# acg-team/ProGraphMSA

Measured on AMD Instinct MI355X. Metric: DP cell-updates/sec (GCUPS) + wall-clock on 256 seqs × 1000 aa, WAG, higher is better.
Workload: dtype f32

## Files before the change

### include/pgm_hip.h

```cpp
#ifndef PGM_HIP_H_
#define PGM_HIP_H_

#include <stdint.h>
#include <stddef.h>

#ifdef __cplusplus
extern "C" {
#endif

#define PGM_OK 0
#define PGM_ERR_INVALID 1
#define PGM_ERR_DEVICE 2
#define PGM_ERR_BACKTRACK 3
#define PGM_ERR_NOMEM 4

#define PGM_GAP 0xFFFFFFFFu


typedef struct pgm_graph {
    uint32_t n;
    uint32_t dim;
    const double *sites;
    const int32_t *e_rowptr;
    const uint32_t *e_col;
// ... 55 lines not shown
                               const pgm_graph *const *g2, const pgm_model *const *model,
                               const pgm_scores *scores, const pgm_site_ref *res1,
                               const pgm_site_ref *res2, pgm_align_out *out);
int pgm_align_batch_run(pgm_ctx *ctx, pgm_align_batch *b);
int pgm_align_batch_fetch(pgm_ctx *ctx, pgm_align_batch *b, pgm_align_out *out);
void pgm_align_batch_destroy(pgm_ctx *ctx, pgm_align_batch *b);
uint64_t pgm_align_batch_cells(const pgm_align_batch *b);
int pgm_align_batch_time(pgm_ctx *ctx, pgm_align_batch *b, int reps, float *ms_prep,
                         float *ms_emission, float *ms_fill, float *ms_traceback);
int pgm_align_batch_stage_times(pgm_align_batch *b, int reset, float *ms_prep, float *ms_emission, float *ms_fill,
                                uint32_t *launches);
int pgm_align_batch_job_times(pgm_ctx *ctx, pgm_align_batch *b, uint64_t *ticks);
int pgm_align_batch_test_stall(pgm_align_batch *b, uint32_t job, uint32_t band, uint32_t spin_limit);
int pgm_test_cu_shares(uint32_t cus, double lean_cost, uint32_t nlean, double band_cost, uint32_t nbands, double rest_cost,
                       uint32_t nrest, uint32_t ncrit, double longest_chain, uint32_t *out4);
int pgm_align_batch_read_matrices(pgm_ctx *ctx, pgm_align_batch *b, uint32_t job, float *M,
                                  float *X, float *Y, float *W, float *S);

int pgm_nw_pairs_batch(pgm_ctx *ctx, uint32_t dim, const int32_t *score, int32_t gap_open,
                       int32_t gap_extend, uint32_t nseq, const int8_t *syms,
                       const uint32_t *offs, uint32_t npairs, const uint32_t *pi,
                       const uint32_t *pj, int32_t *counts, uint32_t *gaps);
#define PGM_NW_REDUCED 1u
int pgm_nw_pairs_submit(pgm_ctx *ctx, uint32_t dim, const int32_t *score, int32_t gap_open,
                        int32_t gap_extend, uint32_t nseq, const int8_t *syms,
                        const uint32_t *offs, uint32_t npairs, const uint32_t *pi,
                        const uint32_t *pj, uint32_t flags, int32_t *counts, uint32_t *gaps, int *ticket);
int pgm_nw_pairs_wait(pgm_ctx *ctx, int ticket);
float pgm_nw_last_kernel_ms(pgm_ctx *ctx);
void *pgm_host_alloc(size_t bytes);
// ... 80 lines not shown
```

### prographmsa_amd/__init__.py

```python
import ctypes as C
import os

_HERE = os.path.dirname(os.path.abspath(__file__))
LIB_PATH = os.path.join(_HERE, "lib", "libpgm_hip.so")
PGMSA_PATH = os.path.join(_HERE, "bin", "pgmsa")

PGM_OK, PGM_ERR_INVALID, PGM_ERR_DEVICE, PGM_ERR_BACKTRACK, PGM_ERR_NOMEM = 0, 1, 2, 3, 4
PGM_GAP = 0xFFFFFFFF
PGM_BATCH_KEEP_MATRICES = 1
PGM_NW_REDUCED = 1
PGM_MERGE_RESIDENT = 1


class pgm_graph(C.Structure):
    _fields_ = [("n", C.c_uint32), ("dim", C.c_uint32), ("sites", C.POINTER(C.c_double)),
                ("e_rowptr", C.POINTER(C.c_int32)), ("e_col", C.POINTER(C.c_uint32)), ("e_val", C.POINTER(C.c_float)),
                ("r_rowptr", C.POINTER(C.c_int32)), ("r_col", C.POINTER(C.c_uint32)), ("r_units", C.POINTER(C.c_uint32))]


class pgm_model(C.Structure):
    _fields_ = [("M", C.POINTER(C.c_double)), ("pi", C.POINTER(C.c_double))]


class pgm_scores(C.Structure):
# ... 26 lines not shown
    _fields_ = [("masks", C.POINTER(C.c_uint64)), ("children", C.POINTER(C.c_uint32)), ("nleaves", C.c_uint32), ("ncols", C.c_uint32)]


class pgm_wls_job(C.Structure):
    _fields_ = [("label", C.POINTER(C.c_int8)), ("offset", C.POINTER(C.c_double)), ("nsub", C.c_uint32)]


class pgm_align_out(C.Structure):
    _fields_ = [("score", C.c_float), ("n_tr_indels", C.c_uint32), ("len", C.c_uint32), ("status", C.c_int32),
                ("map1", C.POINTER(C.c_uint32)), ("map2", C.POINTER(C.c_uint32))]


EXPORTS = [
    "pgm_device_count", "pgm_ctx_create", "pgm_ctx_destroy", "pgm_last_error", "pgm_ctx_device_info",
    "pgm_align_graphs_batch", "pgm_align_batch_create", "pgm_align_batch_create_ex", "pgm_align_batch_create_res", "pgm_align_graphs_batch_res", "pgm_align_batch_run", "pgm_align_batch_fetch",
    "pgm_align_batch_destroy", "pgm_align_batch_cells", "pgm_align_batch_test_stall", "pgm_test_cu_shares", "pgm_align_batch_stage_times", "pgm_align_batch_job_times", "pgm_align_batch_time", "pgm_align_batch_read_matrices",
    "pgm_nw_pairs_batch", "pgm_nw_pairs_submit", "pgm_nw_pairs_wait", "pgm_nw_last_kernel_ms", "pgm_host_alloc", "pgm_host_free", "pgm_csprofile_load", "pgm_csprofile_create_batch", "pgm_csprofile_create_batch_res",
    "pgm_csprofile_last_kernel_ms", "pgm_mldist_batch", "pgm_prealigned_counts_batch", "pgm_kmer_cosine", "pgm_dist_last_kernel_ms",
    "pgm_merge_profiles_batch", "pgm_merge_profiles_batch_ex", "pgm_resident_reset", "pgm_resident_onehot", "pgm_resident_import", "pgm_merge_last_kernel_ms",
    "pgm_gapmask_extend_batch", "pgm_gap_parsimony_batch", "pgm_parsimony_last_kernel_ms",
    "pgm_wls_load", "pgm_wls_pair_sums_batch", "pgm_wls_last_kernel_ms", "pgm_wls_last_launches",
]


def _load():
    if not os.path.exists(LIB_PATH):
        raise ImportError("libpgm_hip.so is not built (%s); run `python -c 'import __graft_entry__ as g; g.build()'` "
                          "— there is no CPU fallback for the hot path" % LIB_PATH)
    lib = C.CDLL(LIB_PATH)
    vp, u32, i32 = C.c_void_p, C.c_uint32, C.c_int32
    PG, PM = C.POINTER(C.POINTER(pgm_graph)), C.POINTER(C.POINTER(pgm_model))
# ... 2 lines not shown
        "pgm_ctx_create": (C.c_int, [C.c_int, C.POINTER(vp)]),
        "pgm_ctx_destroy": (None, [vp]),
        "pgm_last_error": (C.c_char_p, []),
        "pgm_ctx_device_info": (C.c_int, [vp, C.c_char_p, C.c_size_t, C.POINTER(C.c_int)]),
        "pgm_align_graphs_batch": (C.c_int, [vp, u32, PG, PG, PM, C.POINTER(pgm_scores), C.POINTER(pgm_align_out)]),
        "pgm_align_batch_create": (C.c_int, [vp, u32, PG, PG, PM, C.POINTER(pgm_scores), C.POINTER(vp)]),
        "pgm_align_batch_create_ex": (C.c_int, [vp, u32, PG, PG, PM, C.POINTER(pgm_scores), u32, C.POINTER(vp)]),
        "pgm_align_batch_create_res": (C.c_int, [vp, u32, PG, PG, PM, C.POINTER(pgm_scores), u32, C.POINTER(pgm_site_ref), C.POINTER(pgm_site_ref), C.POINTER(vp)]),
        "pgm_align_graphs_batch_res": (C.c_int, [vp, u32, PG, PG, PM, C.POINTER(pgm_scores), C.POINTER(pgm_site_ref), C.POINTER(pgm_site_ref), C.POINTER(pgm_align_out)]),
        "pgm_align_batch_run": (C.c_int, [vp, vp]),
        "pgm_align_batch_fetch": (C.c_int, [vp, vp, C.POINTER(pgm_align_out)]),
        "pgm_align_batch_destroy": (None, [vp, vp]),
        "pgm_align_batch_cells": (C.c_uint64, [vp]),
        "pgm_align_batch_test_stall": (C.c_int, [vp, u32, u32, u32]),
        "pgm_test_cu_shares": (C.c_int, [u32, C.c_double, u32, C.c_double, u32, C.c_double, u32, u32, C.c_double, C.POINTER(C.c_uint32)]),
        "pgm_align_batch_stage_times": (C.c_int, [vp, C.c_int] + [C.POINTER(C.c_float)] * 3 + [C.POINTER(u32)]),
        "pgm_align_batch_job_times": (C.c_int, [vp, vp, C.POINTER(C.c_uint64)]),
        "pgm_align_batch_time": (C.c_int, [vp, vp, C.c_int] + [C.POINTER(C.c_float)] * 4),
        "pgm_align_batch_read_matrices": (C.c_int, [vp, vp, u32] + [C.POINTER(C.c_float)] * 5),
        "pgm_nw_pairs_batch": (C.c_int, [vp, u32, C.POINTER(i32), i32, i32, u32, C.POINTER(C.c_int8), C.POINTER(u32), u32,
                                         C.POINTER(u32), C.POINTER(u32), C.POINTER(i32), C.POINTER(u32)]),
        "pgm_nw_pairs_submit": (C.c_int, [vp, u32, C.POINTER(i32), i32, i32, u32, C.POINTER(C.c_int8), C.POINTER(u32), u32,
                                          C.POINTER(u32), C.POINTER(u32), u32, C.POINTER(i32), C.POINTER(u32), C.POINTER(C.c_int)]),
        "pgm_nw_pairs_wait": (C.c_int, [vp, C.c_int]),
        "pgm_host_alloc": (vp, [C.c_size_t]),
        "pgm_host_free": (None, [vp]),
        "pgm_nw_last_kernel_ms": (C.c_float, [vp]),
        "pgm_csprofile_load": (C.c_int, [vp, u32, u32] + [C.POINTER(C.c_double)] * 3),
        "pgm_csprofile_create_batch": (C.c_int, [vp, u32, C.POINTER(C.c_int8), C.POINTER(u32)] + [C.POINTER(C.c_double)] * 4
                                       + [C.POINTER(C.c_uint64)]),
# ... 63 lines not shown
```

### prographmsa_amd/csrc/pgm_align_kernels.h

```cpp
#ifndef PGM_ALIGN_KERNELS_H_
#define PGM_ALIGN_KERNELS_H_

#include <hip/hip_runtime.h>
#include <math.h>
#include <type_traits>
#include "pgm_device.h"

#define PGM_NEG_INF (-INFINITY)

__device__ __forceinline__ float pgm_ls_log_add(float x, float add) {
    const float a = 2.44247459618085927548717403238913328776812604856113966238617812902399112761292613763080658235564f;
    const float b = -4.2040783745848554315883301529007786406310628696382695994938550046831869207082846248658671f;
    const float c = -0.72123729809042963774358701619456664388406302428056983119308906451199556380646306f;
    const uint32_t bits = __float_as_uint(x);
    const float e = (float)((int32_t)(bits >> 23) - 126);
    const float d = __uint_as_float(((bits << 9) >> 9) ^ 0x3f000000u);
    float t = __fdiv_rn(b, __fsub_rn(d, c));
    const float u = __fadd_rn(e, a);
    t = __fadd_rn(t, add);
    t = __fadd_rn(t, u);
    return t;
}

__device__ __forceinline__ float pgm_emission_finish(float num, float ay, float bx, float match_init) {
// ... 138 lines not shown
    return ((size_t)b * J.tsteps + (x + l)) * 64u + l;
}
__device__ __forceinline__ float4 pgm_load_cell(const PgmJob &J, uint32_t y, uint32_t x) {
    return J.cells[pgm_cell_index(J, y, x)];
}

__device__ __forceinline__ float pgm_dpp_wave_shr1(float src, float lane0_value) {
    return __int_as_float(__builtin_amdgcn_update_dpp(__float_as_int(lane0_value), __float_as_int(src), 0x138, 0xf, 0xf, false));
}

#define PGM_GLOBAL __attribute__((address_space(1)))
typedef float pgm_v4f __attribute__((ext_vector_type(4)));
template <class T> __device__ __forceinline__ T pgm_gld(const T *p) { return *(const PGM_GLOBAL T *)(uintptr_t)p; }
#define PGM_EM_TB 4
template <int DP, int RB>
__global__ void __launch_bounds__(4 * PGM_ROWS) pgm_emission_skew_kernel(const PgmJob *__restrict__ jobs) {
    typedef float pgm_v2f __attribute__((ext_vector_type(2)));
    constexpr int NT = DP / 4;
    constexpr int COLS = 64 + PGM_EM_TB * PGM_BLOCK - PGM_HALO - 1;
    constexpr int STR = DP + 1;
    __shared__ pgm_v2f tp[(COLS + 1) * STR];
    __shared__ float bq[COLS];
    const PgmJob &J = jobs[blockIdx.z];
    const uint32_t tb0 = blockIdx.x * PGM_EM_TB;
    const uint32_t rsh = J.rshift, nvb = J.nb << rsh;
    if (tb0 >= J.nblk || 4u * RB * blockIdx.y >= nvb) return;
    if (J.tabhdr && pgm_gld(J.tabhdr) == 0) return;
    auto row_of = [&](uint32_t v, uint32_t lane_) { return ((((v >> rsh) << 6) + lane_) << rsh) | (v & ((1u << rsh) - 1u)); };
    auto sblock_of = [&](uint32_t v, uint32_t tb_) { return ((((size_t)(v >> rsh) * J.nblk + tb_) << rsh) | (v & ((1u << rsh) - 1u))); };
    const uint32_t t0 = tb0 * PGM_BLOCK;
    const int cbase = (int)t0 - 63;
    if ((DP == 20 || DP == 4) && RB == 1) {
        constexpr int TE = DP + 1;
        float *const tab = (float *)tp;
        static_assert(COLS * TE <= (COLS + 1) * STR * 2, "score table must fit the column staging area");
        static_assert(DP > 20 || TE <= 32, "row classes must fit As");
        __shared__ float As[32];
        const uint32_t fb0 = 4u * blockIdx.y + threadIdx.x / PGM_ROWS;
// ... 2395 lines not shown
```

### prographmsa_amd/csrc/pgm_capi.hip

```cpp
#include <hip/hip_runtime.h>

#include <algorithm>
#include <cmath>
#include <cstdio>
#include <thread>
#include <atomic>
#include <chrono>
#include <queue>
#include <cstdlib>
#include <cstring>
#include <numeric>
#include <mutex>
#include <string>
#include <unordered_set>
#include <vector>
#include <sys/mman.h>

#include "pgm_align_kernels.h"
#include "pgm_crit_kernels.h"
#include "pgm_nw_kernels.h"
#include "pgm_csprofile_kernels.h"
#include "pgm_dist_kernels.h"
#include "pgm_merge_kernels.h"
#include "pgm_parsimony_kernels.h"
// ... 116 lines not shown
    PgmItem *d_items = nullptr;
    uint32_t *d_lean = nullptr;
    uint32_t nlean = 0, nlean_workers = 0;
    uint32_t nbands = 0, nband_workers = 0;
    uint32_t nbands_narrow = 0, nwide_workers = 0;
    PgmItem *d_bands = nullptr;
    unsigned long long *d_times = nullptr;
    hipEvent_t ev_join_b = nullptr;
    bool crit_c3 = false, rest_c3 = false;
    uint32_t ncrit = 0, ncrit_workers = 0, ntb_c = 0;
    hipEvent_t ev_join_c = nullptr;
    uint32_t ntb_b = 0, ntb_b_workers = 0;
    uint32_t lq_off = 0, ntb = 0, ntb_workers = 0;
    int2 *d_tblist = nullptr;
    hipEvent_t ev_fork = nullptr, ev_join = nullptr;
    uint32_t test_spin_limit = 0, test_stall_job = 0xFFFFFFFFu, test_stall_band = 0;
    double acc_ms[3] = {0, 0, 0};
    uint32_t acc_n = 0;
    bool ev_pending = false;
    uint32_t nitems = 0;
    uint32_t nworkers = 0, maxnblk = 0;
    PgmJob *d_jobs = nullptr;
    uint32_t *d_order = nullptr;
    int *d_tabhdr = nullptr;
    size_t in_bytes = 0, work_bytes = 0, cell_bytes = 0, out_bytes = 0;
    std::vector<size_t> res_off, map1_off, map2_off;
    hipEvent_t ev[5] = {nullptr, nullptr, nullptr, nullptr, nullptr};
};

extern "C" {
// ... 362 lines not shown
        ctx->sc_host[slot] = nullptr; ctx->sc_host_bytes[slot] = 0;
        const size_t want = bytes + bytes / 4;
        hipError_t e = pinned_alloc(want, &ctx->sc_host[slot]);
        if (e != hipSuccess) return e;
        ctx->sc_host_bytes[slot] = want;
    }
    *out = ctx->sc_host[slot];
    return hipSuccess;
}
static hipError_t scratch_events(pgm_ctx *ctx) {
    for (int k = 0; k < 2; ++k)
        if (!ctx->sc_ev[k]) { hipError_t e = hipEventCreate(&ctx->sc_ev[k]); if (e != hipSuccess) return e; }
    return hipSuccess;
}

struct CuShares { uint32_t lean, band, crit, rest, rest_need; double t_goal, fl, fb; };
static CuShares cu_shares(uint32_t cus, double lean_cost, uint32_t nlean, double band_cost, uint32_t nbands, double rest_cost, uint32_t nrest, uint32_t ncrit, double rsweep) {
    CuShares r = {0u, 0u, 0u, 0u, 0u, 0.0, 1.0, 1.0};
    cus = std::max(1u, cus);
    const uint32_t queues = (nlean != 0) + (nbands != 0) + (nrest != 0);
    if (ncrit != 0 && cus > queues) r.crit = std::min(std::min(ncrit, cus / 2u), cus - queues);
    const uint32_t cap = std::max(1u, cus - r.crit);
    const double sum = (nlean ? lean_cost : 0.0) + (nbands ? band_cost : 0.0) + (nrest ? rest_cost : 0.0);
    const double t_par = std::max(1e-3, sum / cap);
    r.t_goal = std::max(std::max(rsweep, t_par), 1e-3);
    const double w = std::min(1.0, std::max(0.0, (rsweep / t_par - 1.0) / 0.5));
    r.fl = 1.0 - 0.4 * w; r.fb = 1.0 - 0.25 * w;
    auto need = [](double cost, double t, uint32_t most) { return (uint32_t)std::min<double>(most, std::max(1.0, std::ceil(cost / t))); };
    const uint32_t band_most = (nbands + PGM_WAVES - 1) / PGM_WAVES;
    uint32_t lean = nlean ? need(lean_cost, r.fl * r.t_goal, nlean) : 0u, band = nbands ? need(band_cost, r.fb * r.t_goal, band_most) : 0u;
    uint32_t rest = nrest ? need(rest_cost, r.t_goal, nrest) : 0u;
    if (lean + band + rest > cap) {
        const double scale = (double)cap / (double)(lean + band + rest);
        auto cut = [&](uint32_t v) { return v ? std::max(1u, (uint32_t)std::floor(v * scale)) : 0u; };
        lean = cut(lean); band = cut(band); rest = cut(rest);
        while (lean + band + rest > cap) {
            uint32_t *big = &rest; if (band > *big) big = &band; if (lean > *big) big = &lean;
            if (*big <= 1u) break;
            --*big;
        }
    }
    r.rest_need = rest;
    const uint32_t left = cap > lean + band + rest ? cap - lean - band - rest : 0u;
    if (nrest) rest = std::min(nrest, rest + left);
    else if (nbands) band = std::min(band_most, band + left);
    else if (nlean) lean = std::min(nlean, lean + left);
// ... 15 lines not shown
    hipError_t e;
    for (uint32_t i = 0; i < b->njobs; ++i) ((PgmJob::Result *)(b->h_out + b->res_off[i]))->status = PGM_STATUS_PENDING;
    if (timed && (e = hipEventRecord(b->ev[0], s)) != hipSuccess) return e;
    if (b->maxdim <= 4) {
        const size_t prep_lds = ((size_t)b->maxdim * b->maxdim + b->maxdim + 256 * ((size_t)b->maxdim + 1)) * sizeof(float);
        hipLaunchKernelGGL((pgm_prep_kernel<4, 256>), dim3(b->njobs, 2, (b->maxn + 255) / 256), dim3(256), prep_lds, s, b->d_jobs, b->d_sync, (uint32_t)b->sync_ints);
    } else if (b->maxdim <= 20) {
        const size_t prep_lds = ((size_t)b->maxdim * b->maxdim + b->maxdim + 256 * ((size_t)b->maxdim + 1)) * sizeof(float);
        hipLaunchKernelGGL((pgm_prep_kernel<20, 256>), dim3(b->njobs, 2, (b->maxn + 255) / 256), dim3(256), prep_lds, s, b->d_jobs, b->d_sync, (uint32_t)b->sync_ints);
    } else {
        const size_t prep_lds = ((size_t)b->maxdim * b->maxdim + b->maxdim + 64 * ((size_t)b->maxdim + 1)) * sizeof(float);
        hipLaunchKernelGGL((pgm_prep_kernel<64, 64>), dim3(b->njobs, 2, (b->maxn + 63) / 64), dim3(64), prep_lds, s, b->d_jobs, b->d_sync, (uint32_t)b->sync_ints);
    }
    if ((e = hipGetLastError()) != hipSuccess) return e;
    if (timed && (e = hipEventRecord(b->ev[1], s)) != hipSuccess) return e;
    const dim3 eg((b->maxnblk + PGM_EM_TB - 1) / PGM_EM_TB, (b->maxnb + 3) / 4, b->njobs);
    if (b->maxdim <= 4) hipLaunchKernelGGL((pgm_emission_skew_kernel<4, 1>), eg, dim3(4 * PGM_ROWS), 0, s, b->d_jobs);
    else if (b->maxdim <= 20) hipLaunchKernelGGL((pgm_emission_skew_kernel<20, 1>), eg, dim3(4 * PGM_ROWS), 0, s, b->d_jobs);
    else hipLaunchKernelGGL((pgm_emission_skew_kernel<64, 1>), eg, dim3(4 * PGM_ROWS), 0, s, b->d_jobs);
    if ((e = hipGetLastError()) != hipSuccess) return e;
    if (timed && (e = hipEventRecord(b->ev[2], s)) != hipSuccess) return e;
    const uint32_t spin_limit = b->test_spin_limit ? b->test_spin_limit : PGM_SPIN_LIMIT, stall_job = b->test_stall_job, stall_band = b->test_stall_band;
    const bool fork = b->nlean != 0;
    const bool bandk = b->nbands != 0;
    const bool tbk = (b->nitems != 0 || bandk) && (b->ntb + b->ntb_c + b->ntb_b) != 0;
    const bool critk = b->ncrit != 0;
    if ((fork || bandk || critk) && (e = hipEventRecord(b->ev_fork, s)) != hipSuccess) return e;
    if (critk && (e = hipStreamWaitEvent(ctx->stream4, b->ev_fork, 0)) != hipSuccess) return e;
    if (fork && (e = hipStreamWaitEvent(ctx->stream2, b->ev_fork, 0)) != hipSuccess) return e;
    if (bandk && (e = hipStreamWaitEvent(ctx->stream3, b->ev_fork, 0)) != hipSuccess) return e;
    const uint32_t nrest = b->nitems - b->ncrit;
    hipStream_t sc = critk ? s : ctx->stream4, sr = critk ? ctx->stream4 : s;
    auto sweep = [&](hipStream_t st, uint32_t workers, const PgmItem *list, uint32_t n, bool c3, uint32_t ticket_off) {
        if (c3) hipLaunchKernelGGL(pgm_crit_kernel, dim3(workers), dim3(64 * PGM_C3_WAVES), 0, st, b->d_jobs, list, n, b->d_sync, spin_limit, stall_job, stall_band, ticket_off);
        else hipLaunchKernelGGL(pgm_fill_kernel, dim3(workers), dim3(64 * PGM_WAVES), 0, st, b->d_jobs, list, n, b->d_sync, spin_limit, stall_job, stall_band, ticket_off);
    };
    auto tracebacks = [&](hipStream_t st, uint32_t workers, uint32_t first, uint32_t n, uint32_t lq_off, uint32_t sybase) {
        hipLaunchKernelGGL(pgm_tb_kernel, dim3(workers), dim3(64 * PGM_WAVES), 0, st, b->d_jobs, b->d_tblist + first, n, b->d_sync, b->test_spin_limit, lq_off, sybase, 1u);
    };
    if (critk) sweep(sc, b->ncrit_workers, b->d_items, b->ncrit, b->crit_c3, (uint32_t)PGM_SY_CRIT_TICKET);
    if (nrest != 0) sweep(sr, b->nworkers, b->d_items + b->ncrit, nrest, b->rest_c3, 1u);
    if ((e = hipGetLastError()) != hipSuccess) return e;
    if (fork) {
        hipLaunchKernelGGL((pgm_lean_kernel<2>), dim3(b->nlean_workers), dim3(64 * PGM_WAVES), 0, ctx->stream2, b->d_jobs, b->d_lean, b->nlean, b->d_sync, spin_limit);
        if ((e = hipGetLastError()) != hipSuccess) return e;
    }
    const uint32_t njp = (b->njobs + 3u) / 4u * 4u;
    if (bandk) {
        hipLaunchKernelGGL(pgm_band_kernel, dim3(b->nband_workers), dim3(64 * PGM_WAVES), 0, ctx->stream3, b->d_jobs, b->d_bands, b->nbands_narrow, b->nbands, b->nband_workers - b->nwide_workers, b->d_sync, spin_limit, stall_job, stall_band);
        if ((e = hipGetLastError()) != hipSuccess) return e;
        if (tbk && b->ntb_b) tracebacks(ctx->stream3, b->ntb_b_workers, b->ntb + b->ntb_c, b->ntb_b, b->lq_off + njp, 8u);
        if ((e = hipGetLastError()) != hipSuccess) return e;
        if ((e = hipEventRecord(b->ev_join_b, ctx->stream3)) != hipSuccess) return e;
    }
    if (critk) {
        if (tbk && b->ntb_c) tracebacks(sc, b->ncrit_workers, b->ntb, b->ntb_c, b->lq_off + 2 * njp, 16u);
        if ((e = hipGetLastError()) != hipSuccess) return e;
    }
    if (tbk && b->ntb) {
        tracebacks(sr, b->ntb_workers, 0u, b->ntb, b->lq_off, 0u);
        if ((e = hipGetLastError()) != hipSuccess) return e;
// ... 2 lines not shown
    if (bandk && (e = hipStreamWaitEvent(s, b->ev_join_b, 0)) != hipSuccess) return e;
    if (critk && (e = hipStreamWaitEvent(s, b->ev_join_c, 0)) != hipSuccess) return e;
    if (fork && ((e = hipEventRecord(b->ev_join, ctx->stream2)) != hipSuccess || (e = hipStreamWaitEvent(s, b->ev_join, 0)) != hipSuccess)) return e;
    if (timed && (e = hipEventRecord(b->ev[3], s)) != hipSuccess) return e;
    if (timed && (e = hipEventRecord(b->ev[4], s)) != hipSuccess) return e;
    return hipSuccess;
}
}

extern "C" {

int pgm_test_cu_shares(uint32_t cus, double lean_cost, uint32_t nlean, double band_cost, uint32_t nbands, double rest_cost, uint32_t nrest,
                       uint32_t ncrit, double longest_chain, uint32_t *out4) {
    if (!out4) return fail(PGM_ERR_INVALID, "null argument");
    const CuShares r = cu_shares(cus, lean_cost, nlean, band_cost, nbands, rest_cost, nrest, ncrit, longest_chain);
    out4[0] = r.lean; out4[1] = r.band; out4[2] = r.crit; out4[3] = r.rest;
    return PGM_OK;
}

int pgm_align_batch_create(pgm_ctx *ctx, uint32_t njobs, const pgm_graph *const *g1, const pgm_graph *const *g2,
                           const pgm_model *const *model, const pgm_scores *scores, pgm_align_batch **out) {
    return pgm_align_batch_create_ex(ctx, njobs, g1, g2, model, scores, 0u, out);
}

int pgm_align_batch_create_ex(pgm_ctx *ctx, uint32_t njobs, const pgm_graph *const *g1, const pgm_graph *const *g2,
                              const pgm_model *const *model, const pgm_scores *scores, uint32_t flags, pgm_align_batch **out) {
    return pgm_align_batch_create_res(ctx, njobs, g1, g2, model, scores, flags, nullptr, nullptr, out);
}

int pgm_align_batch_create_res(pgm_ctx *ctx, uint32_t njobs, const pgm_graph *const *g1, const pgm_graph *const *g2,
// ... 67 lines not shown
    L.sync_ints += 3 * (((size_t)njobs + 3) / 4 * 4);
    const size_t sync_ints = L.sync_ints;
    b->sync_ints = sync_ints;
    hipError_t alloc_err = hipSuccess, alloc_host_err = hipSuccess;
    uint8_t *h_out_dev = nullptr;
    const bool cprof = getenv("PGM_HOST_PROFILE") != nullptr;
    auto now_ms = []() { return std::chrono::duration<double, std::milli>(std::chrono::steady_clock::now().time_since_epoch()).count(); };
    const double tc0 = now_ms();
    double tc_alloc = 0, tc_hostalloc = 0, tc_slot[6] = {0, 0, 0, 0, 0, 0};
    size_t total_bands = 0;
    for (uint32_t i = 0; i < njobs; ++i) total_bands += b->jobs[i].nb;
    DevLayout SM;
    const size_t small_sync = SM.take(sync_ints * sizeof(int)), small_jobs = SM.take(sizeof(PgmJob) * std::max(1u, njobs)),
                 small_order = SM.take(4 * (size_t)std::max(1u, njobs)), small_items = SM.take(sizeof(PgmItem) * std::max<size_t>(1, total_bands)),
                 small_lean = SM.take(4 * (size_t)std::max(1u, njobs)), small_tblist = SM.take(8 * (size_t)std::max(1u, njobs)),
                 small_bands = SM.take(sizeof(PgmItem) * std::max<size_t>(1, total_bands)), small_times = SM.take(16 * (size_t)std::max(1u, njobs) + 16);
    bool any_lean = false;
    for (uint32_t i = 0; i < njobs; ++i) any_lean = any_lean || (b->jobs[i].lean && !b->jobs[i].keep_cells);
    const size_t small_tabhdr = SM.take(any_lean ? 4 * (size_t)PGM_TAB_HDR * njobs : 16);
    const size_t small_bytes = SM.bytes;
    std::atomic<int> alloc_state(0);
    std::atomic<int> upload_err((int)hipSuccess);
    std::thread alloc_thread([&]() {
        const double ta0 = now_ms();
        hipError_t e2 = hipSetDevice(ctx->device);
        double tprev = ta0;
        auto lap = [&](int k) { const double t = now_ms(); tc_slot[k] = t - tprev; tprev = t; };
        if (e2 == hipSuccess) { e2 = cache_take(ctx, pgm_ctx::C_IN, b->in_bytes, (void **)&b->d_in, &b->cap[pgm_ctx::C_IN]); lap(0); }
        if (e2 == hipSuccess) { e2 = cache_take(ctx, pgm_ctx::C_WORK, b->work_bytes, (void **)&b->d_work, &b->cap[pgm_ctx::C_WORK]); lap(1); }
        if (e2 == hipSuccess) { e2 = cache_take(ctx, pgm_ctx::C_CELLS, b->cell_bytes, (void **)&b->d_cells, &b->cap[pgm_ctx::C_CELLS]); lap(2); }
        if (e2 == hipSuccess) { e2 = cache_take(ctx, pgm_ctx::C_OUT, b->out_bytes, (void **)&b->d_out, &b->cap[pgm_ctx::C_OUT]); lap(3); }
        if (e2 == hipSuccess) { e2 = cache_take(ctx, pgm_ctx::C_S, b->s_bytes, (void **)&b->d_S, &b->cap[pgm_ctx::C_S]); lap(4); }
        if (e2 == hipSuccess) { e2 = cache_take(ctx, pgm_ctx::C_SMALL, small_bytes, (void **)&b->d_small, &b->cap[pgm_ctx::C_SMALL]); lap(5); }
        if (e2 == hipSuccess) {
            b->d_sync = (int *)(b->d_small + small_sync);
            b->d_jobs = (PgmJob *)(b->d_small + small_jobs);
            b->d_order = (uint32_t *)(b->d_small + small_order);
            b->d_items = (PgmItem *)(b->d_small + small_items);
            b->d_lean = (uint32_t *)(b->d_small + small_lean);
            b->d_tblist = (int2 *)(b->d_small + small_tblist);
            b->d_bands = (PgmItem *)(b->d_small + small_bands);
            b->d_times = (unsigned long long *)(b->d_small + small_times);
            b->d_tabhdr = any_lean ? (int *)(b->d_small + small_tabhdr) : nullptr;
        }
        alloc_err = e2;
        alloc_state.store(e2 == hipSuccess ? 1 : -1, std::memory_order_release);
        tc_alloc = now_ms() - ta0;
        if (e2 == hipSuccess) {
            hipError_t e3 = cache_take(ctx, pgm_ctx::C_HOST, b->out_bytes + 64, (void **)&b->h_out, &b->cap[pgm_ctx::C_HOST]);
            if (e3 == hipSuccess) b->h_flag = (int *)(b->h_out + (b->out_bytes + 15) / 16 * 16);
            if (e3 == hipSuccess) e3 = hipHostGetDevicePointer((void **)&h_out_dev, b->h_out, 0);
            alloc_host_err = e3;
        }
        tc_hostalloc = now_ms() - ta0 - tc_alloc;
    });
    hipError_t e;
    if ((e = cache_take(ctx, pgm_ctx::C_HIN, b->in_bytes, (void **)&b->h_in, &b->cap[pgm_ctx::C_HIN])) != hipSuccess) {
// ... 140 lines not shown
        J.S = (float *)(b->d_S + o.S);
        J.prog = b->d_sync + o.prog;
        J.ltab = (uint16_t *)(w + o.ltab); J.lready = b->d_sync + o.lready; J.lrows = o.lrows; J.lcols = o.lcols;
        J.times = b->d_times + 2 * (size_t)i;
    }
    b->order.resize(njobs);
    std::iota(b->order.begin(), b->order.end(), 0u);
    std::stable_sort(b->order.begin(), b->order.end(), [&](uint32_t x, uint32_t y) {
        return (uint64_t)b->jobs[x].n1 * b->jobs[x].n2 > (uint64_t)b->jobs[y].n1 * b->jobs[y].n2;
    });
    std::vector<PgmItem> items;
    std::vector<uint32_t> lean_list;
    double lean_cost = 0.0, other_cost = 0.0;
    uint32_t capacity = (uint32_t)ctx->prop.multiProcessorCount;
    std::vector<PgmItem> bands;
    if (njobs) {
        struct Item { double rem, dur, gap; uint32_t job, band, count; };
        std::vector<std::vector<Item>> per_job(njobs), per_job_b(njobs), per_job_c(njobs), per_job_w(njobs);
        std::vector<double> chain_of(njobs, 0.0);
        const double lag = PGM_ROWS + 3.0 * PGM_BLOCK;
        constexpr double tau_x = 0.65, tau_c = 0.45, tau_2 = 0.6, eager = 0.7;
        constexpr double tau_3 = 0.42;
        constexpr double tau_l = 0.34;
        size_t total = 0, total_b = 0, total_w = 0;
        double rmax = 1.0, rsweep = 1.0;
        for (uint32_t q = 0; q < njobs; ++q) {
            const uint32_t i = b->order[q];
            const PgmJob &J = b->jobs[i];
            const double tau = J.crit3 ? tau_3 : (J.mode2 ? tau_2 : (J.has_extras ? tau_x : tau_c));
            const double tb = (J.has_extras ? 0.3 : 0.2) * (double)(J.n1 + J.n2);
// ... 27 lines not shown
        double wide_cost = 0.0;
        for (uint32_t i = 0; i < njobs; ++i) {
            for (const Item &it : per_job[i]) other_cost += it.dur;
            for (const Item &it : per_job_b[i]) band_cost += it.dur / PGM_WAVES;
            for (const Item &it : per_job_w[i]) wide_cost += it.dur / PGM_WIDE_WAVES;
        }
        band_cost += wide_cost;
        size_t total_c = 0;
        if (total != 0) {
            uint32_t ncj = 0, nrestj = 0;
            for (uint32_t i = 0; i < njobs; ++i) if (!per_job[i].empty()) { if (chain_of[i] >= 0.85 * rsweep) ++ncj; else ++nrestj; }
            if (ncj != 0 && nrestj != 0)
                for (uint32_t i = 0; i < njobs; ++i)
                    if (!per_job[i].empty() && chain_of[i] >= 0.85 * rsweep) { total_c += per_job[i].size(); for (const Item &it : per_job[i]) crit_cost += it.dur; }
        }
        CuShares sh = cu_shares(capacity, lean_cost, (uint32_t)lean_list.size(), band_cost, (uint32_t)(total_b + 2 * total_w), other_cost - crit_cost, (uint32_t)(total - total_c), (uint32_t)total_c, rsweep);
        if (total_c != 0 && sh.crit == 0) {
            total_c = 0; crit_cost = 0.0;
            sh = cu_shares(capacity, lean_cost, (uint32_t)lean_list.size(), band_cost, (uint32_t)(total_b + 2 * total_w), other_cost, (uint32_t)total, 0u, rsweep);
        }
        if (total_c != 0)
            for (uint32_t i = 0; i < njobs; ++i)
                if (!per_job[i].empty() && chain_of[i] >= 0.85 * rsweep) per_job_c[i].swap(per_job[i]);
        total -= total_c;
        const double t_goal = sh.t_goal;
        uint32_t lean_cus = sh.lean, band_cus = sh.band, crit_cus = sh.crit;
        if (lean_cus) { const uint32_t rounds = ((uint32_t)lean_list.size() + lean_cus - 1u) / lean_cus; lean_cus = ((uint32_t)lean_list.size() + rounds - 1u) / rounds; }
        b->nlean = (uint32_t)lean_list.size();
        b->nlean_workers = lean_cus;
        auto simulate = [&](std::vector<std::vector<Item>> &pj, size_t count, uint32_t workers, std::vector<PgmItem> &out) -> double {
            out.clear();
            double end = 0.0;
            typedef std::pair<double, uint32_t> TE;
            std::priority_queue<double, std::vector<double>, std::greater<double>> free_at;
            for (uint32_t w = 0; w < std::max(1u, workers); ++w) free_at.push(0.0);
            std::priority_queue<TE> ready;
            std::priority_queue<TE, std::vector<TE>, std::greater<TE>> pending;
            std::vector<uint32_t> next(njobs, 0);
// ... 27 lines not shown
                if (total_b == 0) return cus;
                const uint32_t w = (uint32_t)std::lround(cus * wide_cost / band_cost);
                return std::max(1u, std::min(cus > 1u ? cus - 1u : 1u, w));
            };
            auto run = [&](uint32_t cus) {
                wide_cus = split(cus);
                const uint32_t ncus = cus > wide_cus ? cus - wide_cus : (total_b ? 1u : 0u);
                double e = 0.0;
                if (total_b) e = simulate(per_job_b, total_b, ncus * PGM_WAVES, bands);
                if (total_w) e = std::max(e, simulate(per_job_w, total_w, wide_cus * PGM_WIDE_WAVES, bands_w));
                return e;
            };
            if (total != 0) {
                for (int it = 0; it < 3 && band_cus < most; ++it) {
                    band_end = run(band_cus);
                    if (band_end <= sh.fb * t_goal) break;
                    band_cus = std::min(most, std::max(band_cus + 1u, (uint32_t)std::ceil(band_cus * std::min(2.0, band_end / (sh.fb * t_goal)))));
                }
            }
            band_cus = std::max(1u, std::min<uint32_t>(std::min(band_cus, most), (uint32_t)((total_b + PGM_WAVES - 1) / PGM_WAVES + (total_w + PGM_WIDE_WAVES - 1) / PGM_WIDE_WAVES)));
            if (total_b && total_w) band_cus = std::max(band_cus, 2u);
            band_end = run(band_cus);
            if (total_b == 0) bands.clear();
            b->nbands_narrow = (uint32_t)(total_b ? bands.size() : 0);
            bands.insert(bands.end(), bands_w.begin(), bands_w.end());
        }
        if (total_b + total_w != 0) {
            uint32_t nbj = 0;
            for (uint32_t i = 0; i < njobs; ++i) nbj += (!per_job_b[i].empty() || !per_job_w[i].empty());
            const uint32_t most = std::max(band_cus, band_cus + (sh.rest > sh.rest_need ? sh.rest - sh.rest_need : 0u));
            if (nbj > band_cus) {
                const uint32_t rounds = (nbj + band_cus - 1u) / band_cus, want = rounds > 1u ? (nbj + rounds - 2u) / (rounds - 1u) : band_cus;
// ... 52 lines not shown
        b->ntb_workers = std::max(1u, (b->ntb_b || b->ntb_c) ? b->nworkers : all_cus);
        b->ntb_b_workers = std::max(1u, (b->ntb || b->ntb_c) ? b->nband_workers : all_cus);
        if (tblist.empty()) tblist.push_back(make_int2(0, 0));
    }
    if ((e = (hipError_t)upload_err.load()) != hipSuccess ||
        (e = hipMemcpyAsync(b->d_tblist, tblist.data(), 8 * tblist.size(), hipMemcpyHostToDevice, ctx->stream)) != hipSuccess ||
        (e = hipMemcpyAsync(b->d_jobs, b->jobs.data(), sizeof(PgmJob) * njobs, hipMemcpyHostToDevice, ctx->stream)) != hipSuccess ||
        (e = hipMemcpyAsync(b->d_order, b->order.data(), 4 * (size_t)njobs, hipMemcpyHostToDevice, ctx->stream)) != hipSuccess ||
        (e = hipMemcpyAsync(b->d_items, items.data(), sizeof(PgmItem) * items.size(), hipMemcpyHostToDevice, ctx->stream)) != hipSuccess ||
        (e = hipMemcpyAsync(b->d_lean, lean_list.data(), 4 * lean_list.size(), hipMemcpyHostToDevice, ctx->stream)) != hipSuccess ||
        (e = hipMemcpyAsync(b->d_bands, bands.data(), sizeof(PgmItem) * bands.size(), hipMemcpyHostToDevice, ctx->stream)) != hipSuccess ||
        (e = classify_lean_jobs(ctx, b)) != hipSuccess ||
        (e = hipStreamSynchronize(ctx->stream)) != hipSuccess) {
        pgm_align_batch_destroy(ctx, b);
        return fail(PGM_ERR_DEVICE, std::string("upload: ") + hipGetErrorString(e));
    }
    for (int k = 0; k < 5; ++k) (void)hipEventCreate(&b->ev[k]);
    (void)hipEventCreateWithFlags(&b->ev_fork, hipEventDisableTiming);
    (void)hipEventCreateWithFlags(&b->ev_join, hipEventDisableTiming);
    (void)hipEventCreateWithFlags(&b->ev_join_b, hipEventDisableTiming);
    (void)hipEventCreateWithFlags(&b->ev_join_c, hipEventDisableTiming);
    if (cprof)
        fprintf(stderr, "    create: sizes %.2f ms, pinned input block %.2f, flatten %.2f, wait for the allocations %.2f (device %.2f, pinned results %.2f), work list %.2f, upload of %.1f MB %.2f\n",
                tc0 - tcs, tc1 - tc0, tc2 - tc1, tc3 - tc2, tc_alloc, tc_hostalloc, tc4 - tc3, b->in_bytes / 1e6, now_ms() - tc4);
    if (cprof)
        fprintf(stderr, "    device buffers: inputs %.1f MB %.2f ms, work %.1f MB %.2f, cells %.1f MB %.2f, results %.1f MB %.2f, S %.1f MB %.2f, small %.2f\n",
                b->in_bytes / 1e6, tc_slot[0], b->work_bytes / 1e6, tc_slot[1], b->cell_bytes / 1e6, tc_slot[2], b->out_bytes / 1e6, tc_slot[3], b->s_bytes / 1e6, tc_slot[4], tc_slot[5]);
    *out = b;
    return PGM_OK;
}
// ... 230 lines not shown
```

Before: 80.27.

## Launch emission per job groups with trimmed grids, skip lean jobs without tables

The single emission launch over all jobs with a max-sized grid is replaced by per-queue launches over a device job list. Jobs are sorted by grid size and optionally split into two launches to cut empty blocks, and lean jobs whose classification shows no table are dropped from emission. The CU share solver also gains optional per-queue head-start terms, though the callers still pass null. This adds a blocking device-to-host copy of the class verdicts at batch creation and more kernel launches per run.

```diff
diff --git a/include/pgm_hip.h b/include/pgm_hip.h
--- a/include/pgm_hip.h
+++ b/include/pgm_hip.h
@@ -93,6 +93,8 @@
 int pgm_align_batch_test_stall(pgm_align_batch *b, uint32_t job, uint32_t band, uint32_t spin_limit);
 int pgm_test_cu_shares(uint32_t cus, double lean_cost, uint32_t nlean, double band_cost, uint32_t nbands, double rest_cost,
                        uint32_t nrest, uint32_t ncrit, double longest_chain, uint32_t *out4);
+int pgm_test_cu_shares_ex(uint32_t cus, double lean_cost, uint32_t nlean, double band_cost, uint32_t nbands, double rest_cost,
+                          uint32_t nrest, uint32_t ncrit, double longest_chain, const double *head4, uint32_t *out4);
 int pgm_align_batch_read_matrices(pgm_ctx *ctx, pgm_align_batch *b, uint32_t job, float *M,
                                   float *X, float *Y, float *W, float *S);
 
diff --git a/prographmsa_amd/__init__.py b/prographmsa_amd/__init__.py
--- a/prographmsa_amd/__init__.py
+++ b/prographmsa_amd/__init__.py
@@ -64,7 +64,7 @@
 EXPORTS = [
     "pgm_device_count", "pgm_ctx_create", "pgm_ctx_destroy", "pgm_last_error", "pgm_ctx_device_info",
     "pgm_align_graphs_batch", "pgm_align_batch_create", "pgm_align_batch_create_ex", "pgm_align_batch_create_res", "pgm_align_graphs_batch_res", "pgm_align_batch_run", "pgm_align_batch_fetch",
-    "pgm_align_batch_destroy", "pgm_align_batch_cells", "pgm_align_batch_test_stall", "pgm_test_cu_shares", "pgm_align_batch_stage_times", "pgm_align_batch_job_times", "pgm_align_batch_time", "pgm_align_batch_read_matrices",
+    "pgm_align_batch_destroy", "pgm_align_batch_cells", "pgm_align_batch_test_stall", "pgm_test_cu_shares", "pgm_test_cu_shares_ex", "pgm_align_batch_stage_times", "pgm_align_batch_job_times", "pgm_align_batch_time", "pgm_align_batch_read_matrices",
     "pgm_nw_pairs_batch", "pgm_nw_pairs_submit", "pgm_nw_pairs_wait", "pgm_nw_last_kernel_ms", "pgm_host_alloc", "pgm_host_free", "pgm_csprofile_load", "pgm_csprofile_create_batch", "pgm_csprofile_create_batch_res",
     "pgm_csprofile_last_kernel_ms", "pgm_mldist_batch", "pgm_prealigned_counts_batch", "pgm_kmer_cosine", "pgm_dist_last_kernel_ms",
     "pgm_merge_profiles_batch", "pgm_merge_profiles_batch_ex", "pgm_resident_reset", "pgm_resident_onehot", "pgm_resident_import", "pgm_merge_last_kernel_ms",
@@ -97,6 +97,7 @@
         "pgm_align_batch_cells": (C.c_uint64, [vp]),
         "pgm_align_batch_test_stall": (C.c_int, [vp, u32, u32, u32]),
         "pgm_test_cu_shares": (C.c_int, [u32, C.c_double, u32, C.c_double, u32, C.c_double, u32, u32, C.c_double, C.POINTER(C.c_uint32)]),
+        "pgm_test_cu_shares_ex": (C.c_int, [u32, C.c_double, u32, C.c_double, u32, C.c_double, u32, u32, C.c_double, C.POINTER(C.c_double), C.POINTER(C.c_uint32)]),
         "pgm_align_batch_stage_times": (C.c_int, [vp, C.c_int] + [C.POINTER(C.c_float)] * 3 + [C.POINTER(u32)]),
         "pgm_align_batch_job_times": (C.c_int, [vp, vp, C.POINTER(C.c_uint64)]),
         "pgm_align_batch_time": (C.c_int, [vp, vp, C.c_int] + [C.POINTER(C.c_float)] * 4),
diff --git a/prographmsa_amd/csrc/pgm_align_kernels.h b/prographmsa_amd/csrc/pgm_align_kernels.h
--- a/prographmsa_amd/csrc/pgm_align_kernels.h
+++ b/prographmsa_amd/csrc/pgm_align_kernels.h
@@ -176,14 +176,14 @@
 template <class T> __device__ __forceinline__ T pgm_gld(const T *p) { return *(const PGM_GLOBAL T *)(uintptr_t)p; }
 #define PGM_EM_TB 4
 template <int DP, int RB>
-__global__ void __launch_bounds__(4 * PGM_ROWS) pgm_emission_skew_kernel(const PgmJob *__restrict__ jobs) {
+__global__ void __launch_bounds__(4 * PGM_ROWS) pgm_emission_skew_kernel(const PgmJob *__restrict__ jobs, const uint32_t *__restrict__ list) {
     typedef float pgm_v2f __attribute__((ext_vector_type(2)));
     constexpr int NT = DP / 4;
     constexpr int COLS = 64 + PGM_EM_TB * PGM_BLOCK - PGM_HALO - 1;
     constexpr int STR = DP + 1;
     __shared__ pgm_v2f tp[(COLS + 1) * STR];
     __shared__ float bq[COLS];
-    const PgmJob &J = jobs[blockIdx.z];
+    const PgmJob &J = jobs[list[blockIdx.z]];
     const uint32_t tb0 = blockIdx.x * PGM_EM_TB;
     const uint32_t rsh = J.rshift, nvb = J.nb << rsh;
     if (tb0 >= J.nblk || 4u * RB * blockIdx.y >= nvb) return;
diff --git a/prographmsa_amd/csrc/pgm_capi.hip b/prographmsa_amd/csrc/pgm_capi.hip
--- a/prographmsa_amd/csrc/pgm_capi.hip
+++ b/prographmsa_amd/csrc/pgm_capi.hip
@@ -154,6 +154,10 @@
     uint32_t lq_off = 0, ntb = 0, ntb_workers = 0;
     int2 *d_tblist = nullptr;
     hipEvent_t ev_fork = nullptr, ev_join = nullptr;
+    enum { EM_CRIT, EM_REST, EM_BAND, EM_LEAN, EM_QUEUES };
+    struct EmLaunch { uint32_t first, n, gx, gy; };
+    std::vector<EmLaunch> em[EM_QUEUES];
+    uint32_t *d_emlist = nullptr;
     uint32_t test_spin_limit = 0, test_stall_job = 0xFFFFFFFFu, test_stall_band = 0;
     double acc_ms[3] = {0, 0, 0};
     uint32_t acc_n = 0;
@@ -546,22 +550,37 @@
     return hipSuccess;
 }
 
-struct CuShares { uint32_t lean, band, crit, rest, rest_need; double t_goal, fl, fb; };
-static CuShares cu_shares(uint32_t cus, double lean_cost, uint32_t nlean, double band_cost, uint32_t nbands, double rest_cost, uint32_t nrest, uint32_t ncrit, double rsweep) {
-    CuShares r = {0u, 0u, 0u, 0u, 0u, 0.0, 1.0, 1.0};
+struct CuShares { uint32_t lean, band, crit, rest, rest_need; double t_goal, fl, fb, band_by; };
+static CuShares cu_shares(uint32_t cus, double lean_cost, uint32_t nlean, double band_cost, uint32_t nbands, double rest_cost, uint32_t nrest, uint32_t ncrit, double rsweep,
+                          const double *head = nullptr) {
+    CuShares r = {0u, 0u, 0u, 0u, 0u, 0.0, 1.0, 1.0, 0.0};
     cus = std::max(1u, cus);
     const uint32_t queues = (nlean != 0) + (nbands != 0) + (nrest != 0);
     if (ncrit != 0 && cus > queues) r.crit = std::min(std::min(ncrit, cus / 2u), cus - queues);
     const uint32_t cap = std::max(1u, cus - r.crit);
     const double sum = (nlean ? lean_cost : 0.0) + (nbands ? band_cost : 0.0) + (nrest ? rest_cost : 0.0);
-    const double t_par = std::max(1e-3, sum / cap);
-    r.t_goal = std::max(std::max(rsweep, t_par), 1e-3);
-    const double w = std::min(1.0, std::max(0.0, (rsweep / t_par - 1.0) / 0.5));
+    auto head_of = [&](int k, bool work) { return (head && work && head[k] > 0.0 && std::isfinite(head[k])) ? head[k] : 0.0; };
+    const double hl = head_of(0, nlean != 0), hb = head_of(1, nbands != 0), hc = head_of(2, r.crit != 0), hr = head_of(3, nrest != 0);
+    const double t_par0 = std::max(1e-3, sum / cap);
+    double t_par = t_par0;
+    if (hl != 0.0 || hb != 0.0 || hr != 0.0) {
+        double lo = std::max(1e-3, t_par0 - std::max(hl, std::max(hb, hr))), hi = t_par0;
+        for (int it = 0; it < 48; ++it) {
+            const double t = 0.5 * (lo + hi);
+            const double want = (nlean ? lean_cost / (t + hl) : 0.0) + (nbands ? band_cost / (t + hb) : 0.0) + (nrest ? rest_cost / (t + hr) : 0.0);
+            if (want > (double)cap) lo = t; else hi = t;
+        }
+        t_par = hi;
+    }
+    const double chain = std::max(0.0, rsweep - (r.crit ? hc : (nrest ? hr : hb)));
+    r.t_goal = std::max(std::max(chain, t_par), 1e-3);
+    const double w = std::min(1.0, std::max(0.0, (rsweep / t_par0 - 1.0) / 0.5));
     r.fl = 1.0 - 0.4 * w; r.fb = 1.0 - 0.25 * w;
+    r.band_by = r.fb * r.t_goal + hb;
     auto need = [](double cost, double t, uint32_t most) { return (uint32_t)std::min<double>(most, std::max(1.0, std::ceil(cost / t))); };
     const uint32_t band_most = (nbands + PGM_WAVES - 1) / PGM_WAVES;
-    uint32_t lean = nlean ? need(lean_cost, r.fl * r.t_goal, nlean) : 0u, band = nbands ? need(band_cost, r.fb * r.t_goal, band_most) : 0u;
-    uint32_t rest = nrest ? need(rest_cost, r.t_goal, nrest) : 0u;
+    uint32_t lean = nlean ? need(lean_cost, r.fl * r.t_goal + hl, nlean) : 0u, band = nbands ? need(band_cost, r.band_by, band_most) : 0u;
+    uint32_t rest = nrest ? need(rest_cost, r.t_goal + hr, nrest) : 0u;
     if (lean + band + rest > cap) {
         const double scale = (double)cap / (double)(lean + band + rest);
         auto cut = [&](uint32_t v) { return v ? std::max(1u, (uint32_t)std::floor(v * scale)) : 0u; };
@@ -607,23 +626,21 @@
     }
     if ((e = hipGetLastError()) != hipSuccess) return e;
     if (timed && (e = hipEventRecord(b->ev[1], s)) != hipSuccess) return e;
-    const dim3 eg((b->maxnblk + PGM_EM_TB - 1) / PGM_EM_TB, (b->maxnb + 3) / 4, b->njobs);
-    if (b->maxdim <= 4) hipLaunchKernelGGL((pgm_emission_skew_kernel<4, 1>), eg, dim3(4 * PGM_ROWS), 0, s, b->d_jobs);
-    else if (b->maxdim <= 20) hipLaunchKernelGGL((pgm_emission_skew_kernel<20, 1>), eg, dim3(4 * PGM_ROWS), 0, s, b->d_jobs);
-    else hipLaunchKernelGGL((pgm_emission_skew_kernel<64, 1>), eg, dim3(4 * PGM_ROWS), 0, s, b->d_jobs);
-    if ((e = hipGetLastError()) != hipSuccess) return e;
-    if (timed && (e = hipEventRecord(b->ev[2], s)) != hipSuccess) return e;
     const uint32_t spin_limit = b->test_spin_limit ? b->test_spin_limit : PGM_SPIN_LIMIT, stall_job = b->test_stall_job, stall_band = b->test_stall_band;
     const bool fork = b->nlean != 0;
     const bool bandk = b->nbands != 0;
     const bool tbk = (b->nitems != 0 || bandk) && (b->ntb + b->ntb_c + b->ntb_b) != 0;
     const bool critk = b->ncrit != 0;
-    if ((fork || bandk || critk) && (e = hipEventRecord(b->ev_fork, s)) != hipSuccess) return e;
-    if (critk && (e = hipStreamWaitEvent(ctx->stream4, b->ev_fork, 0)) != hipSuccess) return e;
-    if (fork && (e = hipStreamWaitEvent(ctx->stream2, b->ev_fork, 0)) != hipSuccess) return e;
-    if (bandk && (e = hipStreamWaitEvent(ctx->stream3, b->ev_fork, 0)) != hipSuccess) return e;
     const uint32_t nrest = b->nitems - b->ncrit;
     hipStream_t sc = critk ? s : ctx->stream4, sr = critk ? ctx->stream4 : s;
+    auto emission = [&](hipStream_t st, int q) {
+        for (const pgm_align_batch::EmLaunch &L : b->em[q]) {
+            const dim3 eg(L.gx, L.gy, L.n);
+            if (b->maxdim <= 4) hipLaunchKernelGGL((pgm_emission_skew_kernel<4, 1>), eg, dim3(4 * PGM_ROWS), 0, st, b->d_jobs, b->d_emlist + L.first);
+            else if (b->maxdim <= 20) hipLaunchKernelGGL((pgm_emission_skew_kernel<20, 1>), eg, dim3(4 * PGM_ROWS), 0, st, b->d_jobs, b->d_emlist + L.first);
+            else hipLaunchKernelGGL((pgm_emission_skew_kernel<64, 1>), eg, dim3(4 * PGM_ROWS), 0, st, b->d_jobs, b->d_emlist + L.first);
+        }
+    };
     auto sweep = [&](hipStream_t st, uint32_t workers, const PgmItem *list, uint32_t n, bool c3, uint32_t ticket_off) {
         if (c3) hipLaunchKernelGGL(pgm_crit_kernel, dim3(workers), dim3(64 * PGM_C3_WAVES), 0, st, b->d_jobs, list, n, b->d_sync, spin_limit, stall_job, stall_band, ticket_off);
         else hipLaunchKernelGGL(pgm_fill_kernel, dim3(workers), dim3(64 * PGM_WAVES), 0, st, b->d_jobs, list, n, b->d_sync, spin_limit, stall_job, stall_band, ticket_off);
@@ -631,13 +648,21 @@
     auto tracebacks = [&](hipStream_t st, uint32_t workers, uint32_t first, uint32_t n, uint32_t lq_off, uint32_t sybase) {
         hipLaunchKernelGGL(pgm_tb_kernel, dim3(workers), dim3(64 * PGM_WAVES), 0, st, b->d_jobs, b->d_tblist + first, n, b->d_sync, b->test_spin_limit, lq_off, sybase, 1u);
     };
+    for (int q = 0; q < pgm_align_batch::EM_QUEUES; ++q) emission(s, q);
+    if ((e = hipGetLastError()) != hipSuccess) return e;
+    if (timed && (e = hipEventRecord(b->ev[2], s)) != hipSuccess) return e;
+    if ((fork || bandk || critk) && (e = hipEventRecord(b->ev_fork, s)) != hipSuccess) return e;
+    if (critk && (e = hipStreamWaitEvent(ctx->stream4, b->ev_fork, 0)) != hipSuccess) return e;
+    if (fork && (e = hipStreamWaitEvent(ctx->stream2, b->ev_fork, 0)) != hipSuccess) return e;
+    if (bandk && (e = hipStreamWaitEvent(ctx->stream3, b->ev_fork, 0)) != hipSuccess) return e;
     if (critk) sweep(sc, b->ncrit_workers, b->d_items, b->ncrit, b->crit_c3, (uint32_t)PGM_SY_CRIT_TICKET);
-    if (nrest != 0) sweep(sr, b->nworkers, b->d_items + b->ncrit, nrest, b->rest_c3, 1u);
     if ((e = hipGetLastError()) != hipSuccess) return e;
     if (fork) {
         hipLaunchKernelGGL((pgm_lean_kernel<2>), dim3(b->nlean_workers), dim3(64 * PGM_WAVES), 0, ctx->stream2, b->d_jobs, b->d_lean, b->nlean, b->d_sync, spin_limit);
         if ((e = hipGetLastError()) != hipSuccess) return e;
     }
+    if (nrest != 0) sweep(sr, b->nworkers, b->d_items + b->ncrit, nrest, b->rest_c3, 1u);
+    if ((e = hipGetLastError()) != hipSuccess) return e;
     const uint32_t njp = (b->njobs + 3u) / 4u * 4u;
     if (bandk) {
         hipLaunchKernelGGL(pgm_band_kernel, dim3(b->nband_workers), dim3(64 * PGM_WAVES), 0, ctx->stream3, b->d_jobs, b->d_bands, b->nbands_narrow, b->nbands, b->nband_workers - b->nwide_workers, b->d_sync, spin_limit, stall_job, stall_band);
@@ -670,6 +695,14 @@
                        uint32_t ncrit, double longest_chain, uint32_t *out4) {
     if (!out4) return fail(PGM_ERR_INVALID, "null argument");
     const CuShares r = cu_shares(cus, lean_cost, nlean, band_cost, nbands, rest_cost, nrest, ncrit, longest_chain);
+    out4[0] = r.lean; out4[1] = r.band; out4[2] = r.crit; out4[3] = r.rest;
+    return PGM_OK;
+}
+
+int pgm_test_cu_shares_ex(uint32_t cus, double lean_cost, uint32_t nlean, double band_cost, uint32_t nbands, double rest_cost, uint32_t nrest,
+                          uint32_t ncrit, double longest_chain, const double *head4, uint32_t *out4) {
+    if (!out4) return fail(PGM_ERR_INVALID, "null argument");
+    const CuShares r = cu_shares(cus, lean_cost, nlean, band_cost, nbands, rest_cost, nrest, ncrit, longest_chain, head4);
     out4[0] = r.lean; out4[1] = r.band; out4[2] = r.crit; out4[3] = r.rest;
     return PGM_OK;
 }
@@ -767,7 +800,8 @@
     const size_t small_sync = SM.take(sync_ints * sizeof(int)), small_jobs = SM.take(sizeof(PgmJob) * std::max(1u, njobs)),
                  small_order = SM.take(4 * (size_t)std::max(1u, njobs)), small_items = SM.take(sizeof(PgmItem) * std::max<size_t>(1, total_bands)),
                  small_lean = SM.take(4 * (size_t)std::max(1u, njobs)), small_tblist = SM.take(8 * (size_t)std::max(1u, njobs)),
-                 small_bands = SM.take(sizeof(PgmItem) * std::max<size_t>(1, total_bands)), small_times = SM.take(16 * (size_t)std::max(1u, njobs) + 16);
+                 small_bands = SM.take(sizeof(PgmItem) * std::max<size_t>(1, total_bands)), small_times = SM.take(16 * (size_t)std::max(1u, njobs) + 16),
+                 small_emlist = SM.take(4 * (size_t)std::max(1u, njobs));
     bool any_lean = false;
     for (uint32_t i = 0; i < njobs; ++i) any_lean = any_lean || (b->jobs[i].lean && !b->jobs[i].keep_cells);
     const size_t small_tabhdr = SM.take(any_lean ? 4 * (size_t)PGM_TAB_HDR * njobs : 16);
@@ -794,6 +828,7 @@
             b->d_tblist = (int2 *)(b->d_small + small_tblist);
             b->d_bands = (PgmItem *)(b->d_small + small_bands);
             b->d_times = (unsigned long long *)(b->d_small + small_times);
+            b->d_emlist = (uint32_t *)(b->d_small + small_emlist);
             b->d_tabhdr = any_lean ? (int *)(b->d_small + small_tabhdr) : nullptr;
         }
         alloc_err = e2;
@@ -964,6 +999,8 @@
     double lean_cost = 0.0, other_cost = 0.0;
     uint32_t capacity = (uint32_t)ctx->prop.multiProcessorCount;
     std::vector<PgmItem> bands;
+    std::vector<uint8_t> em_queue(njobs, (uint8_t)pgm_align_batch::EM_LEAN);
+    auto em_scores = [&](uint32_t i) { const PgmJob &J = b->jobs[i]; return (double)((size_t)J.nb * J.nblk * 64u * PGM_BLOCK << J.rshift); };
     if (njobs) {
         struct Item { double rem, dur, gap; uint32_t job, band, count; };
         std::vector<std::vector<Item>> per_job(njobs), per_job_b(njobs), per_job_c(njobs), per_job_w(njobs);
@@ -1021,14 +1058,17 @@
                 for (uint32_t i = 0; i < njobs; ++i)
                     if (!per_job[i].empty() && chain_of[i] >= 0.85 * rsweep) { total_c += per_job[i].size(); for (const Item &it : per_job[i]) crit_cost += it.dur; }
         }
-        CuShares sh = cu_shares(capacity, lean_cost, (uint32_t)lean_list.size(), band_cost, (uint32_t)(total_b + 2 * total_w), other_cost - crit_cost, (uint32_t)(total - total_c), (uint32_t)total_c, rsweep);
+        const double *head = nullptr;
+        CuShares sh = cu_shares(capacity, lean_cost, (uint32_t)lean_list.size(), band_cost, (uint32_t)(total_b + 2 * total_w), other_cost - crit_cost, (uint32_t)(total - total_c), (uint32_t)total_c, rsweep, head);
         if (total_c != 0 && sh.crit == 0) {
             total_c = 0; crit_cost = 0.0;
-            sh = cu_shares(capacity, lean_cost, (uint32_t)lean_list.size(), band_cost, (uint32_t)(total_b + 2 * total_w), other_cost, (uint32_t)total, 0u, rsweep);
+            sh = cu_shares(capacity, lean_cost, (uint32_t)lean_list.size(), band_cost, (uint32_t)(total_b + 2 * total_w), other_cost, (uint32_t)total, 0u, rsweep, head);
         }
         if (total_c != 0)
             for (uint32_t i = 0; i < njobs; ++i)
                 if (!per_job[i].empty() && chain_of[i] >= 0.85 * rsweep) per_job_c[i].swap(per_job[i]);
+        for (uint32_t i = 0; i < njobs; ++i)
+            if (!b->jobs[i].lean) em_queue[i] = (uint8_t)pgm_align_batch::EM_REST;
         total -= total_c;
         const double t_goal = sh.t_goal;
         uint32_t lean_cus = sh.lean, band_cus = sh.band, crit_cus = sh.crit;
@@ -1086,8 +1126,8 @@
             if (total != 0) {
                 for (int it = 0; it < 3 && band_cus < most; ++it) {
                     band_end = run(band_cus);
-                    if (band_end <= sh.fb * t_goal) break;
-                    band_cus = std::min(most, std::max(band_cus + 1u, (uint32_t)std::ceil(band_cus * std::min(2.0, band_end / (sh.fb * t_goal)))));
+                    if (band_end <= sh.band_by) break;
+                    band_cus = std::min(most, std::max(band_cus + 1u, (uint32_t)std::ceil(band_cus * std::min(2.0, band_end / sh.band_by))));
                 }
             }
             band_cus = std::max(1u, std::min<uint32_t>(std::min(band_cus, most), (uint32_t)((total_b + PGM_WAVES - 1) / PGM_WAVES + (total_w + PGM_WIDE_WAVES - 1) / PGM_WIDE_WAVES)));
@@ -1170,6 +1210,58 @@
         (e = hipStreamSynchronize(ctx->stream)) != hipSuccess) {
         pgm_align_batch_destroy(ctx, b);
         return fail(PGM_ERR_DEVICE, std::string("upload: ") + hipGetErrorString(e));
+    }
+    {
+        std::vector<int> no_table(njobs, 1);
+        if (b->d_tabhdr && njobs &&
+            (e = hipMemcpy2D(no_table.data(), sizeof(int), b->d_tabhdr, sizeof(int) * (size_t)PGM_TAB_HDR, sizeof(int), njobs, hipMemcpyDeviceToHost)) != hipSuccess) {
+            pgm_align_batch_destroy(ctx, b);
+            return fail(PGM_ERR_DEVICE, std::string("class verdicts: ") + hipGetErrorString(e));
+        }
+        std::vector<uint32_t> flat;
+        for (int q = 0; q < pgm_align_batch::EM_QUEUES; ++q) {
+            struct G { uint32_t job, gx, gy; };
+            std::vector<G> g;
+            for (uint32_t k = 0; k < njobs; ++k) {
+                const uint32_t i = b->order[k];
+                const PgmJob &J = b->jobs[i];
+                if (em_queue[i] != q || (J.lean && J.tabhdr && no_table[i] == 0)) continue;
+                g.push_back(G{i, (J.nblk + PGM_EM_TB - 1) / PGM_EM_TB, ((J.nb << J.rshift) + 3u) / 4u});
+            }
+            if (g.empty()) continue;
+            std::stable_sort(g.begin(), g.end(), [](const G &x, const G &y) { return (uint64_t)x.gx * x.gy > (uint64_t)y.gx * y.gy; });
+            const size_t n = g.size();
+            std::vector<uint32_t> sx(n + 1, 0), sy(n + 1, 0);
+            for (size_t k = n; k-- > 0;) { sx[k] = std::max(sx[k + 1], g[k].gx); sy[k] = std::max(sy[k + 1], g[k].gy); }
+            const uint64_t whole = (uint64_t)n * sx[0] * sy[0];
+            uint64_t best = whole; size_t cut = 0;
+            uint32_t px = 0, py = 0;
+            for (size_t k = 1; k < n; ++k) {
+                px = std::max(px, g[k - 1].gx); py = std::max(py, g[k - 1].gy);
+                const uint64_t c = (uint64_t)k * px * py + (uint64_t)(n - k) * sx[k] * sy[k];
+                if (c < best) { best = c; cut = k; }
+            }
+            if (best > whole - whole / 4u) cut = 0;
+            const uint32_t first = (uint32_t)flat.size();
+            for (const G &x : g) flat.push_back(x.job);
+            if (cut) {
+                uint32_t cx = 0, cy = 0;
+                for (size_t k = 0; k < cut; ++k) { cx = std::max(cx, g[k].gx); cy = std::max(cy, g[k].gy); }
+                b->em[q].push_back(pgm_align_batch::EmLaunch{first, (uint32_t)cut, cx, cy});
+            }
+            b->em[q].push_back(pgm_align_batch::EmLaunch{first + (uint32_t)cut, (uint32_t)(n - cut), sx[cut], sy[cut]});
+        }
+        if (!flat.empty() && (e = hipMemcpy(b->d_emlist, flat.data(), 4 * flat.size(), hipMemcpyHostToDevice)) != hipSuccess) {
+            pgm_align_batch_destroy(ctx, b);
+            return fail(PGM_ERR_DEVICE, std::string("upload: ") + hipGetErrorString(e));
+        }
+        if (cprof)
+            for (int q = 0; q < pgm_align_batch::EM_QUEUES; ++q)
+                for (const pgm_align_batch::EmLaunch &L : b->em[q]) {
+                    double sc = 0.0;
+                    for (uint32_t k = 0; k < L.n; ++k) sc += em_scores(flat[L.first + k]);
+                    fprintf(stderr, "    emission, queue %d: %u jobs, grid %u x %u x %u, %.3e scores\n", q, L.n, L.gx, L.gy, L.n, sc);
+                }
     }
     for (int k = 0; k < 5; ++k) (void)hipEventCreate(&b->ev[k]);
     (void)hipEventCreateWithFlags(&b->ev_fork, hipEventDisableTiming);
```

After: 81.52 (median of 6 runs). 1.02x the previous value.
